# allisoneer/zvdb

Measured on NVIDIA B200. Metric: batched search QPS at recall@10 (1M x 128 fp32), higher is better.
Workload: dtype f32

## Files before the change

zvdb_b200/csrc/capi.cu:

```cuda
#include <cstring>
#include <algorithm>
#include <atomic>
#include <cstdio>
#include <cstdlib>
#include <mutex>
#include <new>
#include <string>
#include <vector>

#include "../../include/zvdb_b200.h"
#include "host_graph.hpp"
#include "search_kernel.cuh"
#include "search_team_kernel.cuh"
#include "builder.cuh"
#include "bruteforce.cuh"

namespace zvdb {

static thread_local std::string g_last_error;

static int fail(int code, const std::string &msg) {
    g_last_error = msg;
    return code;
}

#define ZV_CUDA(expr)                                                                            \
    do {                                                                                         \
        cudaError_t e__ = (expr);                                                                \
        if (e__ != cudaSuccess) {                                                                \
            cudaGetLastError();                                                                  \
            return fail(e__ == cudaErrorMemoryAllocation ? ZVDB_ERR_OUT_OF_MEMORY : ZVDB_ERR_CUDA, \
                        std::string(#expr) + ": " + cudaGetErrorString(e__));                    \
        }                                                                                        \
    } while (0)


__global__ void scatter_adj_rows_kernel(uint32_t *__restrict__ adj, const uint32_t *__restrict__ rows,
                                        const uint32_t *__restrict__ ids, uint32_t count, uint32_t m) {
    const uint64_t total = static_cast<uint64_t>(count) * m;
    for (uint64_t i = blockIdx.x * static_cast<uint64_t>(blockDim.x) + threadIdx.x; i < total;
         i += static_cast<uint64_t>(gridDim.x) * blockDim.x) {
        const uint32_t r = static_cast<uint32_t>(i / m), c = static_cast<uint32_t>(i % m);
        adj[static_cast<uint64_t>(ids[r]) * m + c] = rows[i];
    }
}

__global__ void arena_to_f16_kernel(uint2 *__restrict__ dst, const float4 *__restrict__ src, uint64_t r0, uint64_t r1,
                                    uint32_t row_chunks, uint32_t *__restrict__ bad_row) {
    const uint64_t begin = r0 * row_chunks, end = r1 * row_chunks;
    for (uint64_t i = begin + blockIdx.x * static_cast<uint64_t>(blockDim.x) + threadIdx.x; i < end;
         i += static_cast<uint64_t>(gridDim.x) * blockDim.x) {
        const float4 v = src[i];
        const __half2 a = __floats2half2_rn(v.x, v.y), b = __floats2half2_rn(v.z, v.w);
        if (__hisinf(__low2half(a)) | __hisinf(__high2half(a)) | __hisinf(__low2half(b)) | __hisinf(__high2half(b)))
            atomicMin(bad_row, static_cast<uint32_t>(i / row_chunks));
        dst[i] = make_uint2(*reinterpret_cast<const uint32_t *>(&a), *reinterpret_cast<const uint32_t *>(&b));
    }
}

template <typename T>
struct DevBuf {
    T *p = nullptr;
    size_t cap = 0;
    cudaError_t reserve(size_t count) {
        if (count <= cap) return cudaSuccess;
        if (p) cudaFree(p);
// ... 5 lines not shown
    void free_() { if (p) cudaFree(p); p = nullptr; cap = 0; }
};

}

using namespace zvdb;

struct zvdb_index {
    std::mutex mu;
    HostGraph g;
    int device = 0;
    int num_sms = 148;
    size_t smem_optin = 0;
    cudaStream_t stream = nullptr;
    cudaStream_t stream2 = nullptr;
    cudaStream_t stream_in = nullptr;
    cudaEvent_t in_ev[8] = {};
    cudaEvent_t bitmap_ev = nullptr;
    cudaEvent_t bf_ev = nullptr;
    unsigned char *h_stage = nullptr;
    size_t h_stage_cap = 0;
    uint32_t *mailbox_dev = nullptr;
    uint32_t mailbox_seq = 0;
    bool mailbox_armed = false;
    float *d_arena = nullptr;
    uint32_t *d_adj = nullptr;
    uint64_t cap_rows = 0, n_dev = 0;
    uint32_t cap_row_floats = 0, cap_m = 0;
    int storage = ZVDB_STORAGE_F32;
    uint2 *d_arena16 = nullptr;
    uint64_t f16_rows = 0;
    DevBuf<uint32_t> f16_bad;
    DevBuf<float> q_buf, dist_buf;
    DevBuf<uint64_t> ids_buf;
    DevBuf<uint32_t> cnt_buf, pops_buf, evals_buf, scat_rows, scat_ids, bitmap_buf, vlog_buf;
    DevBuf<uint64_t> res_buf;
    DevBuf<uint32_t> gtable_buf;
    DevBuf<float> bf_xhi, bf_xlo, bf_xnorm, bf_qhi, bf_qlo;
    DevBuf<uint64_t> bf_part, bf_glists;
    DevBuf<uint4> bf_segs;
    DevBuf<uint32_t> bf_seg_off;
    uint64_t bf_rows = 0;
    DevBuf<uint8_t> d_level;
    DevBuf<uint32_t> d_upper_base, d_upper_adj;
    DevBuf<uint4> seeds_buf;
    uint64_t upper_uploaded = ~0ull;
    bool descent = false;
    uint32_t visited_mode = 0;
    bool legacy_exchange = false;
    bool bitmap_oom = false;
    bool exchange_blocks = false;
    bool stage_host_buffers = false;
    uint32_t team_mode = 0;
    uint32_t prefetch_mode = 0;
    uint32_t bf_mode = 0;
    uint32_t bf_epilogue = 0;
    bool bf_filter = false;
    std::atomic<uint64_t> launches{0};
};

namespace zvdb {

static int ensure_capacity(zvdb_index *ix, uint64_t rows) {
    const HostGraph &g = ix->g;
    const bool same_layout = ix->cap_row_floats == g.row_floats && ix->cap_m == g.m;
    if (same_layout && rows <= ix->cap_rows) return ZVDB_OK;
    if (!same_layout) {
        ZV_CUDA(cudaDeviceSynchronize());
        cudaFree(ix->d_arena); cudaFree(ix->d_adj);
        ix->d_arena = nullptr; ix->d_adj = nullptr; ix->cap_rows = 0; ix->n_dev = 0; ix->bf_rows = 0;
        ix->cap_row_floats = g.row_floats; ix->cap_m = g.m;
    }
    if (ix->d_arena16) {
        ZV_CUDA(cudaDeviceSynchronize());
        cudaFree(ix->d_arena16); ix->d_arena16 = nullptr; ix->f16_rows = 0;
    }
    uint64_t nc = std::max<uint64_t>(rows, std::max<uint64_t>(ix->cap_rows * 2, 1024));
    float *na = nullptr; uint32_t *nj = nullptr;
    ZV_CUDA(cudaMalloc(&na, nc * g.row_floats * sizeof(float)));
    cudaError_t e = cudaMalloc(&nj, nc * g.m * sizeof(uint32_t));
    if (e != cudaSuccess) { cudaFree(na); ZV_CUDA(e); }
    if (ix->n_dev) {
        ZV_CUDA(cudaMemcpyAsync(na, ix->d_arena, ix->n_dev * g.row_floats * sizeof(float), cudaMemcpyDeviceToDevice, ix->stream));
        ZV_CUDA(cudaMemcpyAsync(nj, ix->d_adj, ix->n_dev * g.m * sizeof(uint32_t), cudaMemcpyDeviceToDevice, ix->stream));
        ZV_CUDA(cudaStreamSynchronize(ix->stream));
    }
    cudaFree(ix->d_arena); cudaFree(ix->d_adj);
    ix->d_arena = na; ix->d_adj = nj; ix->cap_rows = nc;
    return ZVDB_OK;
}

static int sync_device_locked(zvdb_index *ix) {
    HostGraph &g = ix->g;
    if (g.n == 0) return ZVDB_OK;
    if (g.rows_uploaded == g.n && !g.adj_all_dirty && g.dirty.empty()) return ZVDB_OK;
    ZV_CUDA(cudaSetDevice(ix->device));
    if (ix->n_dev) ZV_CUDA(cudaDeviceSynchronize());
    int rc = ensure_capacity(ix, g.n);
    if (rc) return rc;
    ix->f16_rows = std::min<uint64_t>(ix->f16_rows, g.rows_uploaded);
    for (uint64_t r = g.rows_uploaded; r < g.n;) {
        const uint64_t chunk = r / g.rows_per_chunk;
        const uint64_t end = std::min<uint64_t>(g.n, (chunk + 1) * g.rows_per_chunk);
        ZV_CUDA(cudaMemcpyAsync(ix->d_arena + r * g.row_floats, g.point(r), (end - r) * g.row_floats * sizeof(float),
                                cudaMemcpyHostToDevice, ix->stream));
        r = end;
// ... 128 lines not shown
    }
    return cudaGetLastError();
}
template <int ROWF>
static cudaError_t launch_descend_rowf(int metric, int cpl, const SearchParams &p, unsigned grid, cudaStream_t s) {
    switch (metric) {
        case 0: return launch_descend_metric<kMetricL2, ROWF>(cpl, p, grid, s);
        case 1: return launch_descend_metric<kMetricCos, ROWF>(cpl, p, grid, s);
        default: return launch_descend_metric<kMetricDot, ROWF>(cpl, p, grid, s);
    }
}
static cudaError_t launch_descend(bool f16, int metric, int cpl, const SearchParams &p, unsigned grid, cudaStream_t s) {
    return f16 ? launch_descend_rowf<kRowF16>(metric, cpl, p, grid, s) : launch_descend_rowf<kRowF32>(metric, cpl, p, grid, s);
}

template <int CPL, int METRIC, bool ADJC, int MC, int T, int ROWF>
static cudaError_t launch_team_inst3(const SearchParams &p, unsigned grid, size_t smem, cudaStream_t s) {
    auto kern = ROWF == kRowF16 ? search_team_f16_kernel<CPL, METRIC, ADJC, MC, T> : search_team_kernel<CPL, METRIC, ADJC, MC, T>;
    if (smem > 48 * 1024) {
        cudaError_t e = cudaFuncSetAttribute(kern, cudaFuncAttributeMaxDynamicSharedMemorySize, static_cast<int>(smem));
        if (e != cudaSuccess) return e;
    }
    kern<<<grid, T, smem, s>>>(p);
    return cudaGetLastError();
}
template <int CPL, int METRIC, int ROWF>
static cudaError_t launch_team_inst(bool adjc, unsigned threads, const SearchParams &p, unsigned grid, size_t smem, cudaStream_t s) {
    if (threads == 128) return launch_team_inst3<CPL, METRIC, false, 0, 128, ROWF>(p, grid, smem, s);
    if (adjc && p.m == 16) return launch_team_inst3<CPL, METRIC, true, 16, 256, ROWF>(p, grid, smem, s);
    return adjc ? launch_team_inst3<CPL, METRIC, true, 0, 256, ROWF>(p, grid, smem, s) : launch_team_inst3<CPL, METRIC, false, 0, 256, ROWF>(p, grid, smem, s);
}
template <int METRIC, int ROWF>
static cudaError_t launch_team_metric(int cpl, bool adjc, unsigned threads, const SearchParams &p, unsigned grid, size_t smem, cudaStream_t s) {
    switch (cpl) {
        case 1: return launch_team_inst<1, METRIC, ROWF>(adjc, threads, p, grid, smem, s);
        case 2: return launch_team_inst<2, METRIC, ROWF>(adjc, threads, p, grid, smem, s);
        case 4: return launch_team_inst<4, METRIC, ROWF>(adjc, threads, p, grid, smem, s);
        case 6: return launch_team_inst<6, METRIC, ROWF>(adjc, threads, p, grid, smem, s);
        case 8: return launch_team_inst<8, METRIC, ROWF>(adjc, threads, p, grid, smem, s);
    }
    return cudaErrorInvalidValue;
}
template <int ROWF>
static cudaError_t launch_team_rowf(int metric, int cpl, bool adjc, unsigned threads, const SearchParams &p, unsigned grid, size_t smem, cudaStream_t s) {
    switch (metric) {
        case 0: return launch_team_metric<kMetricL2, ROWF>(cpl, adjc, threads, p, grid, smem, s);
        case 1: return launch_team_metric<kMetricCos, ROWF>(cpl, adjc, threads, p, grid, smem, s);
        default: return launch_team_metric<kMetricDot, ROWF>(cpl, adjc, threads, p, grid, smem, s);
    }
}
static cudaError_t launch_team(bool f16, int metric, int cpl, bool adjc, unsigned threads, const SearchParams &p, unsigned grid, size_t smem, cudaStream_t s) {
    return f16 ? launch_team_rowf<kRowF16>(metric, cpl, adjc, threads, p, grid, smem, s)
               : launch_team_rowf<kRowF32>(metric, cpl, adjc, threads, p, grid, smem, s);
}

static int plan_visited(const zvdb_index *ix, uint32_t ef) {
    const HostGraph &g = ix->g;
    const uint64_t bound = std::min<uint64_t>(g.n, 1ull + static_cast<uint64_t>(ef) * g.m);
    const uint64_t slots = bound + bound / 4 + 16;
    const uint64_t cand_cap = std::max<uint64_t>(2, next_pow2(ef));
    const uint64_t smem_lists = (((static_cast<uint64_t>(ef) + 1) & ~1ull) + cand_cap) * 8 + kPoolCap * 8 + 32 * 4 + kPoolCap * 4 + 16;
    const uint64_t smem_hash = smem_lists + slots * 4;
    const uint64_t ctas = std::min<uint64_t>(32, (227ull * 1024) / (smem_hash + 1024));
    const uint64_t bitmap_bytes = (g.n + 31) / 32 * 4 * 32ull * static_cast<uint64_t>(ix->num_sms);
    int vis = (smem_hash <= ix->smem_optin && ctas >= 20) ? kVisSmemHash
            : ((bitmap_bytes <= (32ull << 30) && !ix->bitmap_oom) ? kVisGlobalBitmap : kVisGlobalHash);
    if (ix->visited_mode == 1) vis = kVisSmemHash;
    if (ix->visited_mode == 2) vis = kVisGlobalBitmap;
    if (ix->visited_mode == 3) vis = kVisGlobalHash;
    return vis;
}

struct FusedExchange {
    uint32_t *peer_qflags[8];
    const uint32_t *qflags;
    const uint8_t *gather;
    uint64_t block_bytes;
    uint64_t *m_ids; float *m_dist; uint32_t *m_counts;
    uint32_t world, rank, epoch;
    uint8_t *peer_ll[8] = {};
    const uint8_t *ll_local = nullptr;
    uint32_t ll_lines = 0, ll_pitch = 0, ll_nq = 0;
    uint32_t q_per = 0;
    const float *peer_q[8] = {};
    uint32_t *peer_sflags[8] = {};
    const uint32_t *sflags = nullptr;
    uint32_t sflag_pitch = 0;
};

static int launch_search(zvdb_index *ix, const float *d_q, uint64_t nq, uint32_t k, uint32_t ef, uint64_t *d_ids,
                         float *d_dist, uint32_t *d_counts, uint32_t *d_pops, uint32_t *d_evals, uint64_t id_stride,
                         uint64_t id_base, cudaStream_t s, uint8_t *const *peer_blocks = nullptr, uint32_t n_peers = 0,
                         const FusedExchange *fx = nullptr) {
    const HostGraph &g = ix->g;
    if (nq == 0) return ZVDB_OK;
    if (nq > 0x7FFFFFFFull) return fail(ZVDB_ERR_UNSUPPORTED, "nq exceeds 2^31-1 queries per launch");
    const bool f16 = ix->storage == ZVDB_STORAGE_F16 && g.n > 0;
    if (f16 && (fx || n_peers)) return fail(ZVDB_ERR_UNSUPPORTED, "f16 storage: the sharded exchange forms gather fp32 rows only");
    if (f16) {
        int rcf = sync_f16_locked(ix);
        if (rcf) return rcf;
    }
    SearchParams p{};
    p.arena = reinterpret_cast<const float4 *>(ix->d_arena);
    p.arena16 = f16 ? ix->d_arena16 : nullptr;
    p.adj = ix->d_adj;
// ... 16 lines not shown
            ZV_CUDA(ix->seeds_buf.reserve(nq));
        }
        p.seeds = ix->seeds_buf.p;
    }
    const uint32_t chunks_per_lane = (p.row_chunks + 31) / 32;
    if (chunks_per_lane > 8) return fail(ZVDB_ERR_UNSUPPORTED, "dim > 1024 is not built into the search kernel");
    const int cpl = chunks_per_lane <= 1 ? 1 : chunks_per_lane <= 2 ? 2 : chunks_per_lane <= 4 ? 4 : chunks_per_lane <= 6 ? 6 : 8;

    const uint64_t bound = std::max<uint64_t>(1, std::min<uint64_t>(g.n, 1ull + static_cast<uint64_t>(ef) * g.m));
    const uint64_t slots = bound + bound / 4 + 16;
    const uint64_t hash_words = (slots + 3) & ~3ull;
    const uint64_t cand_cap = std::max<uint64_t>(2, next_pow2(ef));
    const uint64_t smem_lists = (((static_cast<uint64_t>(ef) + 1) & ~1ull) + cand_cap) * 8 + kPoolCap * 8 + 32 * 4 + kPoolCap * 4 + 16;
    const uint64_t smem_hash = smem_lists + slots * 4;
    const bool team_auto = ix->team_mode == 0 && ix->visited_mode == 0 && ix->prefetch_mode == 0;
    if (!fx && n_peers == 0 && g.n > 0 && ef > 0 && (team_auto || ix->team_mode >= 2)) {
        const uint32_t ucpl = static_cast<uint32_t>(cpl);
        const uint64_t cap256 = team_cand_cap(ef, g.m, 256), cap128 = team_cand_cap(ef, g.m, 128);
        const uint64_t smem_plain = team_smem_bytes(cap256, ef, hash_words, ucpl, g.m, false);
        const uint64_t smem_cache = team_smem_bytes(cap256, ef, hash_words, ucpl, g.m, true);
        const uint64_t smem_half = team_smem_bytes(cap128, ef, hash_words, ucpl, g.m, false);
        const uint64_t regs256 = cpl <= 1 ? 3 : (cpl <= 4 ? 2 : 1);
        const uint64_t regs128 = cpl <= 1 ? 7 : (cpl <= 2 ? 6 : (cpl <= 4 ? 4 : 2));
        auto resident = [&](uint64_t smem, uint64_t by_regs) { return std::min<uint64_t>(by_regs, (227ull * 1024) / (smem + 1024)) * ix->num_sms; };
        const bool fits_cache = smem_cache <= ix->smem_optin, fits_plain = smem_plain <= ix->smem_optin, fits_half = smem_half <= ix->smem_optin;
        bool use = false, adjc = false;
        unsigned threads = 256;
        uint64_t team_cap = cap256, team_smem = smem_plain;
        if (ix->team_mode == 3) { use = fits_half; threads = 128; }
        else if (ix->team_mode == 2) { use = fits_plain; adjc = fits_cache && (nq <= resident(smem_cache, regs256) || resident(smem_cache, regs256) >= resident(smem_plain, regs256)); }
        else if (fits_cache && nq <= resident(smem_cache, regs256)) { use = true; adjc = true; }
        else if (fits_plain && nq <= resident(smem_plain, regs256)) { use = true; }
        else if (fits_half && nq <= resident(smem_half, regs128)) { use = true; threads = 128; }
        if (adjc) team_smem = smem_cache;
        if (threads == 128) { team_cap = cap128; team_smem = smem_half; }
        if (use) {
            cudaError_t e;
            if (p.seeds) {
                ZV_CUDA(cudaStreamWaitEvent(s, ix->bitmap_ev, 0));
                e = launch_descend(f16, g.metric, cpl, p, static_cast<unsigned>((nq + 3) / 4), s);
                ix->launches++;
                ZV_CUDA(e);
            }
            p.slots = static_cast<uint32_t>(slots); p.hash_words = static_cast<uint32_t>(hash_words);
            p.cand_cap = static_cast<uint32_t>(team_cap);
            if (ix->mailbox_dev && nq == 1) { p.done_flag = ix->mailbox_dev; p.done_seq = ix->mailbox_seq; ix->mailbox_armed = true; }
            e = launch_team(f16, g.metric, cpl, adjc, threads, p, static_cast<unsigned>(nq), static_cast<size_t>(team_smem), s);
            ix->launches++;
            ZV_CUDA(e);
            if (p.seeds) ZV_CUDA(cudaEventRecord(ix->bitmap_ev, s));
            return ZVDB_OK;
        }
    }
    uint64_t merge_smem = 0;
    if (fx) {
        const uint64_t total = static_cast<uint64_t>(fx->world) * k;
        if (total > 4096) return fail(ZVDB_ERR_UNSUPPORTED, "merge: G*k > 4096");
        p.merge_p2 = next_pow2(static_cast<uint32_t>(total));
        merge_smem = (total * 12 + 8 * 4 + 15) & ~15ull;
    }
    auto ctas_for = [](uint64_t smem) { return std::min<uint64_t>(32, (227ull * 1024) / (smem + 1024)); };
    int vis = plan_visited(ix, ef);
    if (vis == kVisGlobalBitmap && ix->visited_mode == 0) {
        const uint64_t resident0 = std::min<uint64_t>(nq, 32ull * ix->num_sms);
        const uint64_t need0 = resident0 * ((g.n + 31) / 32);
        if (need0 > ix->bitmap_buf.cap) {
            cudaError_t eb = ix->bitmap_buf.reserve(need0);
            if (eb == cudaErrorMemoryAllocation) { cudaGetLastError(); ix->bitmap_oom = true; vis = plan_visited(ix, ef); }
            else { ZV_CUDA(eb); ZV_CUDA(cudaMemsetAsync(ix->bitmap_buf.p, 0, ix->bitmap_buf.cap * sizeof(uint32_t), s)); }
        }
    }
    const uint64_t res_cap = (static_cast<uint64_t>(ef) + 1) & ~1ull;
    const bool res_global = vis != kVisSmemHash && ctas_for(smem_lists + merge_smem) < 32;
    uint64_t smem = vis == kVisSmemHash ? smem_hash : (res_global ? smem_lists - res_cap * 8 : smem_lists);
    smem = (smem + 15) & ~15ull;
    p.merge_off = static_cast<uint32_t>(smem);
    smem += merge_smem;
    if (smem > ix->smem_optin) {
        char buf[256];
        snprintf(buf, sizeof buf, "search needs %llu bytes of shared memory per query (ef=%u, m=%u); this device allows %zu. Lower ef.",
                 static_cast<unsigned long long>(smem), ef, g.m, ix->smem_optin);
        return fail(ZVDB_ERR_UNSUPPORTED, buf);
    }
    p.slots = static_cast<uint32_t>(slots); p.hash_words = static_cast<uint32_t>(hash_words);
    p.prefetch = ix->prefetch_mode == 0 ? ((vis != kVisSmemHash && cpl <= 2) ? 1u : 0u) : ix->prefetch_mode - 1u;
    p.cand_cap = static_cast<uint32_t>(cand_cap);
    const uint64_t resident = std::min<uint64_t>(ctas_for(smem), cpl <= 2 ? 32 : 16) * ix->num_sms;
    unsigned grid = static_cast<unsigned>(nq);
    if (vis != kVisSmemHash) {
        grid = static_cast<unsigned>(std::min<uint64_t>(nq, resident));
        ZV_CUDA(cudaStreamWaitEvent(s, ix->bitmap_ev, 0));
        if (vis == kVisGlobalBitmap) {
            const uint64_t bm_words = (g.n + 31) / 32;
            const uint64_t need = grid * bm_words;
            if (need > ix->bitmap_buf.cap) {
                ZV_CUDA(ix->bitmap_buf.reserve(need));
                ZV_CUDA(cudaMemsetAsync(ix->bitmap_buf.p, 0, ix->bitmap_buf.cap * sizeof(uint32_t), s));
            }
            const uint64_t log_cap = (bound + 3) & ~3ull;
            ZV_CUDA(ix->vlog_buf.reserve(grid * log_cap));
            p.gbitmap = ix->bitmap_buf.p; p.glog = ix->vlog_buf.p;
            p.bm_words = static_cast<uint32_t>(bm_words); p.log_cap = static_cast<uint32_t>(log_cap);
        } else {
            const uint64_t need = grid * hash_words;
            if (need > ix->gtable_buf.cap) {
                ZV_CUDA(ix->gtable_buf.reserve(need));
                ZV_CUDA(cudaMemsetAsync(ix->gtable_buf.p, 0xFF, ix->gtable_buf.cap * sizeof(uint32_t), s));
            }
            p.gtable = ix->gtable_buf.p;
        }
        if (res_global) {
            ZV_CUDA(ix->res_buf.reserve(grid * res_cap));
            p.gres = ix->res_buf.p; p.res_cap = static_cast<uint32_t>(res_cap);
        }
// ... 336 lines not shown
    fp.id_stride = id_stride; fp.id_base = id_base;
    fp.row_chunks = pitch / 4; fp.dim = g.dim; fp.nq = p.nq; fp.k = k; fp.kp = p.kp; fp.n_splits = p.n_slots;
    fp.p2 = next_pow2(p.n_slots * p.kp); fp.kk2 = std::max<uint32_t>(2, next_pow2(p.kp));
    const uint32_t cpl_raw = (fp.row_chunks + 31) / 32;
    const int cpl = cpl_raw <= 1 ? 1 : cpl_raw <= 2 ? 2 : cpl_raw <= 4 ? 4 : cpl_raw <= 6 ? 6 : 8;
    const size_t fsmem = (static_cast<size_t>(fp.p2) + fp.kk2) * sizeof(uint64_t);
    cudaError_t e = g.metric == 0 ? launch_bf_final_metric<kMetricL2>(cpl, fp, fsmem, s)
                  : g.metric == 1 ? launch_bf_final_metric<kMetricCos>(cpl, fp, fsmem, s)
                                  : launch_bf_final_metric<kMetricDot>(cpl, fp, fsmem, s);
    ix->launches++;
    ZV_CUDA(e);
    ZV_CUDA(cudaEventRecord(ix->bf_ev, s));
    return ZVDB_OK;
}

}


extern "C" {

const char *zvdb_last_error(void) { return g_last_error.c_str(); }
const char *zvdb_version(void) { return "zvdb_b200 0.1 sm_100a"; }

int zvdb_create(zvdb_index **out, uint32_t dim, uint32_t m, uint32_t ef_construction, int metric, int device) {
    if (!out) return fail(ZVDB_ERR_INVALID, "zvdb_create: out is null");
    *out = nullptr;
    if (m == 0) return fail(ZVDB_ERR_INVALID, "zvdb_create: m must be >= 1");
    if (metric < 0 || metric > 2) return fail(ZVDB_ERR_INVALID, "zvdb_create: unknown metric");
    if (dim > 1024) return fail(ZVDB_ERR_UNSUPPORTED, "zvdb_create: dim > 1024 is not built into the search kernel");
    int count = 0;
    cudaError_t e = cudaGetDeviceCount(&count);
    if (e != cudaSuccess || device < 0 || device >= count) {
        cudaGetLastError();
        return fail(ZVDB_ERR_CUDA, std::string("zvdb_create: no usable CUDA device (there is no CPU fallback): ") +
                                       (e != cudaSuccess ? cudaGetErrorString(e) : "device ordinal out of range"));
    }
    cudaDeviceProp prop{};
    ZV_CUDA(cudaGetDeviceProperties(&prop, device));
    if (prop.major != 10)
        return fail(ZVDB_ERR_CUDA, std::string("zvdb_create: device '") + prop.name + "' is not sm_100; this library carries sm_100a code only");
    zvdb_index *ix = new (std::nothrow) zvdb_index();
    if (!ix) return fail(ZVDB_ERR_OUT_OF_MEMORY, "zvdb_create: out of memory");
    ix->device = device;
    ix->num_sms = prop.multiProcessorCount;
    ix->smem_optin = prop.sharedMemPerBlockOptin;
    ix->g.m = m; ix->g.ef_construction = ef_construction; ix->g.metric = metric;
    if (dim) ix->g.fix_dim(dim);
    e = cudaSetDevice(device);
    if (e == cudaSuccess) e = cudaStreamCreateWithFlags(&ix->stream, cudaStreamNonBlocking);
    if (e == cudaSuccess) e = cudaStreamCreateWithFlags(&ix->stream2, cudaStreamNonBlocking);
    if (e == cudaSuccess) e = cudaStreamCreateWithFlags(&ix->stream_in, cudaStreamNonBlocking);
    for (int i = 0; i < 8 && e == cudaSuccess; ++i) e = cudaEventCreateWithFlags(&ix->in_ev[i], cudaEventDisableTiming);
    if (e == cudaSuccess) e = cudaEventCreateWithFlags(&ix->bitmap_ev, cudaEventDisableTiming);
    if (e == cudaSuccess) e = cudaEventCreateWithFlags(&ix->bf_ev, cudaEventDisableTiming);
    if (e != cudaSuccess) { delete ix; ZV_CUDA(e); }
    *out = ix;
    return ZVDB_OK;
}

void zvdb_destroy(zvdb_index *ix) {
    if (!ix) return;
    cudaSetDevice(ix->device);
    if (ix->stream) { cudaStreamSynchronize(ix->stream); cudaStreamDestroy(ix->stream); }
    if (ix->stream2) { cudaStreamSynchronize(ix->stream2); cudaStreamDestroy(ix->stream2); }
    if (ix->stream_in) { cudaStreamSynchronize(ix->stream_in); cudaStreamDestroy(ix->stream_in); }
    for (int i = 0; i < 8; ++i) if (ix->in_ev[i]) cudaEventDestroy(ix->in_ev[i]);
    if (ix->bitmap_ev) cudaEventDestroy(ix->bitmap_ev);
    if (ix->bf_ev) cudaEventDestroy(ix->bf_ev);
    cudaFree(ix->d_arena); cudaFree(ix->d_adj); cudaFree(ix->d_arena16);
    if (ix->h_stage) cudaFreeHost(ix->h_stage);
    ix->f16_bad.free_();
    ix->q_buf.free_(); ix->dist_buf.free_(); ix->ids_buf.free_(); ix->cnt_buf.free_();
    ix->pops_buf.free_(); ix->evals_buf.free_(); ix->scat_rows.free_(); ix->scat_ids.free_(); ix->bitmap_buf.free_(); ix->vlog_buf.free_(); ix->res_buf.free_(); ix->gtable_buf.free_();
    ix->d_level.free_(); ix->d_upper_base.free_(); ix->d_upper_adj.free_(); ix->seeds_buf.free_();
    ix->bf_xhi.free_(); ix->bf_xlo.free_(); ix->bf_xnorm.free_(); ix->bf_qhi.free_(); ix->bf_qlo.free_(); ix->bf_part.free_(); ix->bf_glists.free_(); ix->bf_segs.free_(); ix->bf_seg_off.free_();
    delete ix;
}

int zvdb_set_level_seed(zvdb_index *ix, uint64_t seed) {
    if (!ix) return fail(ZVDB_ERR_INVALID, "null index");
    std::lock_guard<std::mutex> lk(ix->mu);
    ix->g.rng = seed * 0x9E3779B97F4A7C15ull + 0x243F6A8885A308D3ull;
    return ZVDB_OK;
}

static void to_f32(const void *src, uint64_t count, int dtype, float *dst) {
    if (dtype == 1) { const double *p = static_cast<const double *>(src); for (uint64_t i = 0; i < count; ++i) dst[i] = static_cast<float>(p[i]); }
    else if (dtype == 2) { const int32_t *p = static_cast<const int32_t *>(src); for (uint64_t i = 0; i < count; ++i) dst[i] = static_cast<float>(p[i]); }
    else std::memcpy(dst, src, count * sizeof(float));
}

static int insert_locked(zvdb_index *ix, const void *points_any, uint64_t n, uint32_t dim, const int32_t *levels, int dtype = 0) {
    HostGraph &g = ix->g;
    if (n == 0) return ZVDB_OK;
    if (!points_any) return fail(ZVDB_ERR_INVALID, "insert: null point");
    if (dtype < 0 || dtype > 2) return fail(ZVDB_ERR_INVALID, "insert: dtype must be 0 (f32), 1 (f64) or 2 (i32)");
    if (g.n == 0 && g.chunks.empty()) g.dtype = dtype;
    if (dtype != g.dtype) return fail(ZVDB_ERR_INVALID, "insert: element type differs from the index's (one HNSW(T) holds one T)");
    if (dtype != 0 && g.metric != 0) return fail(ZVDB_ERR_UNSUPPORTED, "insert: f64 / i32 indexes are squared-L2 only, like the reference");
    const float *points = static_cast<const float *>(points_any);
    if (g.dim == 0) {
        if (dim == 0) return fail(ZVDB_ERR_INVALID, "insert: dim must be >= 1");
        if (dim > 1024) return fail(ZVDB_ERR_UNSUPPORTED, "insert: dim > 1024 is not built into the search kernel");
        g.fix_dim(dim);
    }
    if (dim != g.dim) return fail(ZVDB_ERR_DIM_MISMATCH, "Mismatched dimensions in distance calculation");
    cudaSetDevice(ix->device);
    if (dtype == 0) {
        for (uint64_t i = 0; i < n; ++i) {
            if (g.insert(points + i * static_cast<uint64_t>(dim), levels ? levels[i] : -1))
                return fail(ZVDB_ERR_OUT_OF_MEMORY, "insert: out of memory");
        }
        return ZVDB_OK;
    }
    std::vector<float> conv(dim);
    const size_t es = g.elem_size();
    for (uint64_t i = 0; i < n; ++i) {
        const unsigned char *src = static_cast<const unsigned char *>(points_any) + i * static_cast<uint64_t>(dim) * es;
        to_f32(src, dim, dtype, conv.data());
        if (g.insert(conv.data(), levels ? levels[i] : -1, src)) return fail(ZVDB_ERR_OUT_OF_MEMORY, "insert: out of memory");
    }
    return ZVDB_OK;
}

int zvdb_insert(zvdb_index *ix, const float *point, uint32_t dim) {
    if (!ix) return fail(ZVDB_ERR_INVALID, "null index");
// ... 446 lines not shown
    ZV_CUDA(cudaGetLastError());
    const uint64_t total = n * g.m;
    const unsigned blocks = static_cast<unsigned>(std::min<uint64_t>((total + 255) / 256, 148ull * 16));
    count_reverse_kernel<<<blocks, 256, 0, s>>>(d_fw.p, total, d_indeg.p); ix->launches++;
    std::vector<uint32_t> indeg;
    std::vector<uint64_t> off;
    try { indeg.resize(n); off.resize(n + 1); }
    catch (const std::bad_alloc &) { return fail(ZVDB_ERR_OUT_OF_MEMORY, "build: out of memory"); }
    ZV_CUDA(cudaMemcpyAsync(indeg.data(), d_indeg.p, n * sizeof(uint32_t), cudaMemcpyDeviceToHost, s));
    ZV_CUDA(cudaStreamSynchronize(s));
    off[0] = 0;
    for (uint64_t i = 0; i < n; ++i) off[i + 1] = off[i] + indeg[i];
    ZV_CUDA(d_rev.reserve(std::max<uint64_t>(off[n], 1)));
    ZV_CUDA(cudaMemcpyAsync(d_off.p, off.data(), (n + 1) * sizeof(uint64_t), cudaMemcpyHostToDevice, s));
    fill_reverse_kernel<<<blocks, 256, 0, s>>>(d_fw.p, total, g.m, d_off.p, d_indeg.p + n, d_rev.p); ix->launches++;
    bp.rev_off = d_off.p; bp.rev = d_rev.p;
    launch_build(g.metric, cpl, 3, bp, s); ix->launches++;
    ZV_CUDA(cudaGetLastError());
    ZV_CUDA(cudaMemcpyAsync(g.adj0.data(), ix->d_adj, n * g.m * sizeof(uint32_t), cudaMemcpyDeviceToHost, s));
    ZV_CUDA(cudaStreamSynchronize(s));
    return ZVDB_OK;
}

int zvdb_build_from_candidates(zvdb_index *ix, const float *points, uint64_t n, uint32_t dim, const uint32_t *cand,
                               uint32_t K, int cand_on_device) {
    if (!ix || (n && (!points || !cand))) return fail(ZVDB_ERR_INVALID, "null argument");
    if (K == 0 || K > kBuildBuf) return fail(ZVDB_ERR_UNSUPPORTED, "build: K must be in 1..128");
    std::lock_guard<std::mutex> lk(ix->mu);
    HostGraph &g = ix->g;
    if (g.m > 64) return fail(ZVDB_ERR_UNSUPPORTED, "build: m must be <= 64");
    int rc = set_points_locked(ix, points, n, dim, 0);
    if (rc || n == 0) return rc;
    rc = build_from_candidates_locked(ix, n, cand, K, cand_on_device);
    if (rc) {
        const std::string why = g_last_error;
        g.reset_nodes();
        ix->n_dev = 0; ix->bf_rows = 0; ix->f16_rows = 0;
        return fail(rc, why);
    }
    g.rows_uploaded = n; g.dirty.clear(); g.adj_all_dirty = false;
    ix->n_dev = n;
    return ZVDB_OK;
}

int zvdb_sync_device(zvdb_index *ix) {
    if (!ix) return fail(ZVDB_ERR_INVALID, "null index");
    std::lock_guard<std::mutex> lk(ix->mu);
    return sync_device_locked(ix);
}

int zvdb_set_kernel_variant(zvdb_index *ix, uint32_t variant) {
    if (!ix) return fail(ZVDB_ERR_INVALID, "null index");
    const uint32_t width = variant & 3u, vis = (variant >> 2) & 3u, bfm = (variant >> 4) & 3u;
    if (width > 2 || bfm > 2 || variant > 65535 || ((variant >> 8) & 7u) > 4)
        return fail(ZVDB_ERR_INVALID, "variant: bits 0-1 = accepted and ignored (round 1's load-width variants are gone: never faster in any automatically chosen mode), bits 2-3 = visited set 0 auto/1 shared-memory hash/2 global bitmap/3 global hash, bits 4-5 = brute force 0 auto/1 single CTA/2 CTA pair, bit 6 = brute-force TF32 filter, bit 7 = brute-force sorted-list epilogue, bits 8-10 = L2 prefetch 0 auto/1 off/2 rows/3 adjacency/4 both, bit 11 = stage page-locked host buffers through device copies, bit 12 = sharded step as three launches (search, flag, merge) instead of the fused one, bit 13 = fused step through result blocks + release flags instead of 128-byte records, bits 14-15 = one CTA per query for small batches 0 auto/1 never/2 full teams (256 threads) whenever the shape fits/3 half teams (128 threads)");
    std::lock_guard<std::mutex> lk(ix->mu);
    ix->prefetch_mode = (variant >> 8) & 7u; ix->stage_host_buffers = (variant >> 11) & 1u; ix->legacy_exchange = (variant >> 12) & 1u; ix->exchange_blocks = (variant >> 13) & 1u;
    ix->team_mode = (variant >> 14) & 3u;
    ix->visited_mode = vis; ix->bf_mode = bfm; ix->bf_filter = (variant >> 6) & 1u; ix->bf_epilogue = (variant >> 7) & 1u;
    return ZVDB_OK;
}

uint64_t zvdb_kernel_launches(const zvdb_index *ix) { return ix ? ix->launches.load() : 0; }

int zvdb_search_batch_device(zvdb_index *ix, const float *d_queries, uint64_t nq, uint32_t k, uint32_t ef,
                             uint64_t *d_ids, float *d_dist, uint32_t *d_counts, uint32_t *d_pops, uint32_t *d_evals,
                             uint64_t id_stride, uint64_t id_base, void *stream) {
    if (!ix) return fail(ZVDB_ERR_INVALID, "null index");
    if (nq == 0) return ZVDB_OK;
    if (!d_queries || !d_ids || !d_dist || !d_counts) return fail(ZVDB_ERR_INVALID, "search: null buffer");
    if (k == 0) return fail(ZVDB_ERR_INVALID, "search: k must be >= 1");
    if (ef == 0) ef = k;
    if (ef < k) return fail(ZVDB_ERR_INVALID, "search: ef must be >= k");
    std::lock_guard<std::mutex> lk(ix->mu);
    ZV_CUDA(cudaSetDevice(ix->device));
    cudaStream_t s = static_cast<cudaStream_t>(stream);
    if (ix->g.n == 0 || !ix->g.has_entry) {
        ZV_CUDA(cudaMemsetAsync(d_counts, 0, nq * sizeof(uint32_t), s));
        ZV_CUDA(cudaMemsetAsync(d_ids, 0xFF, nq * k * sizeof(uint64_t), s));
        ZV_CUDA(cudaMemsetAsync(d_dist, 0, nq * k * sizeof(float), s));
        if (d_pops) ZV_CUDA(cudaMemsetAsync(d_pops, 0, nq * sizeof(uint32_t), s));
        if (d_evals) ZV_CUDA(cudaMemsetAsync(d_evals, 0, nq * sizeof(uint32_t), s));
        return ZVDB_OK;
    }
    int rc = sync_device_locked(ix);
    if (rc) return rc;
    return launch_search(ix, d_queries, nq, k, ef, d_ids, d_dist, d_counts, d_pops, d_evals, id_stride, id_base, s);
}

int zvdb_search_batch(zvdb_index *ix, const float *queries, uint64_t nq, uint32_t dim, uint32_t k, uint32_t ef,
                      uint64_t *ids, float *dist, uint32_t *counts, uint32_t *pops, uint32_t *evals) {
    if (!ix) return fail(ZVDB_ERR_INVALID, "null index");
    if (nq == 0) return ZVDB_OK;
    if (!queries || !ids || !dist || !counts) return fail(ZVDB_ERR_INVALID, "search: null buffer");
    if (k == 0) return fail(ZVDB_ERR_INVALID, "search: k must be >= 1");
    if (ef == 0) ef = k;
    if (ef < k) return fail(ZVDB_ERR_INVALID, "search: ef must be >= k");
    std::lock_guard<std::mutex> lk(ix->mu);
    ZV_CUDA(cudaSetDevice(ix->device));
    if (ix->g.n == 0 || !ix->g.has_entry) {
        for (uint64_t i = 0; i < nq; ++i) counts[i] = 0;
        for (uint64_t i = 0; i < nq * k; ++i) { ids[i] = ZVDB_INVALID_ID; dist[i] = 0.0f; }
        if (pops) for (uint64_t i = 0; i < nq; ++i) pops[i] = 0;
        if (evals) for (uint64_t i = 0; i < nq; ++i) evals[i] = 0;
        return ZVDB_OK;
    }
    if (dim != ix->g.dim) return fail(ZVDB_ERR_DIM_MISMATCH, "Mismatched dimensions in distance calculation");
    int rc = sync_device_locked(ix);
    if (rc) return rc;
    auto mapped = [](const void *ptr, void **dptr) {
        cudaPointerAttributes a{};
// ... 433 lines not shown
```

zvdb_b200/csrc/search_kernel.cuh:

```cuda
#pragma once
#include <cuda_fp16.h>
#include <type_traits>
#include "common.cuh"

namespace zvdb {

struct SearchParams {
    const float4 *arena;
    const uint32_t *adj;
    const float *queries;
    uint64_t *ids;
    float *dist;
    uint32_t *counts;
    uint32_t *pops;
    uint32_t *evals;
    uint64_t id_stride, id_base;
    uint32_t row_chunks;
    uint32_t m, n, entry, dim, nq, k, ef;
    uint32_t slots;
    uint32_t hash_words;
    uint32_t cand_cap;
    uint8_t *peer_blocks[8];
    uint32_t n_peers;
    const uint8_t *levels;
    const uint32_t *upper_base;
    const uint32_t *upper_adj;
    uint32_t max_level, descent_start;
    uint4 *seeds;
    uint32_t *gbitmap;
    uint32_t *glog;
    uint32_t bm_words, log_cap;
    uint64_t *gres;
    uint32_t res_cap;
    uint32_t prefetch;
    uint32_t *gtable;
    uint32_t *peer_qflags[8];
    const uint32_t *qflags;
    const uint8_t *gather;
    uint64_t block_bytes;
    uint64_t *m_ids; float *m_dist; uint32_t *m_counts;
    uint32_t ex_world, ex_rank, ex_epoch;
    uint32_t merge_p2;
    uint32_t merge_lag;
    uint32_t merge_off;
    uint8_t *peer_ll[8];
    const uint8_t *ll_local;
    uint32_t ll_lines;
    uint32_t ll_pitch;
    uint32_t ll_nq;
    uint32_t q_per;
    const float *peer_q[8];
    uint32_t *peer_sflags[8];
    const uint32_t *sflags;
    uint32_t sflag_pitch;
    uint32_t *done_flag;
    uint32_t done_seq;
    const uint2 *arena16;
};

enum : int { kMetricL2 = 0, kMetricCos = 1, kMetricDot = 2 };
constexpr uint32_t kPoolCap = 64;

enum : int { kRowF32 = 0, kRowF16 = 1 };
template <int ROWF> using RowChunk = std::conditional_t<ROWF == kRowF16, uint2, float4>;
__device__ __forceinline__ float4 chunk_f32(const float4 v) { return v; }
__device__ __forceinline__ float4 chunk_f32(const uint2 w) {
    const float2 a = __half22float2(*reinterpret_cast<const __half2 *>(&w.x));
    const float2 b = __half22float2(*reinterpret_cast<const __half2 *>(&w.y));
    return make_float4(a.x, a.y, b.x, b.y);
}
template <int ROWF> __device__ __forceinline__ RowChunk<ROWF> zero_chunk() {
    if constexpr (ROWF == kRowF16) return make_uint2(0u, 0u); else return make_float4(0.f, 0.f, 0.f, 0.f);
}
template <int ROWF> __device__ __forceinline__ const RowChunk<ROWF> *search_rows(const SearchParams &p) {
    if constexpr (ROWF == kRowF16) return p.arena16; else return p.arena;
}

#ifndef ZVDB_F16_UNROLL
#define ZVDB_F16_UNROLL 1
#endif
template <int CPL, bool WIDE, int ROWF = kRowF32> struct Unroll {
    static constexpr int narrow = CPL <= 1 ? 8 : (CPL <= 2 ? 4 : 2);
    static constexpr int value = (WIDE ? (CPL <= 4 ? narrow * 2 : narrow) : narrow) * (ROWF == kRowF16 ? ZVDB_F16_UNROLL : 1);
};

__device__ __forceinline__ uint64_t pack2(float lo, float hi) {
    uint64_t r; asm("mov.b64 %0, {%1, %2};" : "=l"(r) : "f"(lo), "f"(hi)); return r;
}
__device__ __forceinline__ void unpack2(uint64_t v, float &lo, float &hi) {
    asm("mov.b64 {%0, %1}, %2;" : "=f"(lo), "=f"(hi) : "l"(v));
}
__device__ __forceinline__ uint64_t ffma2(uint64_t a, uint64_t b, uint64_t c) {
    uint64_t d; asm("fma.rn.f32x2 %0, %1, %2, %3;" : "=l"(d) : "l"(a), "l"(b), "l"(c)); return d;
}

struct Chunk2 { uint64_t xy, zw; };

template <int METRIC>
__device__ __forceinline__ uint64_t accumulate_chunk(uint64_t acc, const Chunk2 q, const float4 v) {
    const uint64_t vxy = pack2(v.x, v.y), vzw = pack2(v.z, v.w);
    if (METRIC == kMetricL2) {
        const uint64_t neg1 = pack2(-1.0f, -1.0f);
        const uint64_t dxy = ffma2(vxy, neg1, q.xy);
        const uint64_t dzw = ffma2(vzw, neg1, q.zw);
        acc = ffma2(dxy, dxy, acc);
        acc = ffma2(dzw, dzw, acc);
    } else {
        acc = ffma2(q.xy, vxy, acc);
        acc = ffma2(q.zw, vzw, acc);
    }
// ... 671 lines not shown
```

Before: 23.55 million.

## Add two-queries-per-warp search kernel with small on-chip visited table

Adds a new graph search kernel in which each warp serves two queries, one per 16-lane half. Each half keeps its own candidate list, pool and a small shared-memory visited hash, and spills to a global hash table when linear probing overflows. The kernel is chosen automatically for L2 f32 batches with degree up to 16 when the shared-memory hash path would apply, with the aim of packing more queries per SM and cutting per-query shared memory. The cost is that the two halves run in lockstep, so the warp keeps iterating until both queries finish, and overflow falls back to slower global atomics.

Measured after the change: 16.41 million (median of 6 runs). 0.697x the previous value.

```diff
diff --git a/zvdb_b200/csrc/capi.cu b/zvdb_b200/csrc/capi.cu
--- a/zvdb_b200/csrc/capi.cu
+++ b/zvdb_b200/csrc/capi.cu
@@ -12,6 +12,7 @@
 #include "host_graph.hpp"
 #include "search_kernel.cuh"
 #include "search_team_kernel.cuh"
+#include "search_pair_kernel.cuh"
 #include "builder.cuh"
 #include "bruteforce.cuh"
 
@@ -123,6 +124,11 @@
     bool exchange_blocks = false;
     bool stage_host_buffers = false;
     uint32_t team_mode = 0;
+    bool pair_off = false;
+    bool pair_tiny = false;
+    DevBuf<uint64_t> pair_res2;
+    DevBuf<uint32_t> pair_tab2;
+    cudaEvent_t pair_ev2 = nullptr;
     uint32_t prefetch_mode = 0;
     uint32_t bf_mode = 0;
     uint32_t bf_epilogue = 0;
@@ -357,6 +363,15 @@
 static cudaError_t launch_team(bool f16, int metric, int cpl, bool adjc, unsigned threads, const SearchParams &p, unsigned grid, size_t smem, cudaStream_t s) {
     return f16 ? launch_team_rowf<kRowF16>(metric, cpl, adjc, threads, p, grid, smem, s)
                : launch_team_rowf<kRowF32>(metric, cpl, adjc, threads, p, grid, smem, s);
+}
+
+static cudaError_t launch_pair(const SearchParams &p, unsigned grid, size_t smem, cudaStream_t s) {
+    if (smem > 48 * 1024) {
+        cudaError_t e = cudaFuncSetAttribute(search_pair_kernel<kMetricL2>, cudaFuncAttributeMaxDynamicSharedMemorySize, static_cast<int>(smem));
+        if (e != cudaSuccess) return e;
+    }
+    search_pair_kernel<kMetricL2><<<grid, 32, smem, s>>>(p);
+    return cudaGetLastError();
 }
 
 static int plan_visited(const zvdb_index *ix, uint32_t ef) {
@@ -479,6 +494,43 @@
             return ZVDB_OK;
         }
     }
+    auto ctas_for = [](uint64_t smem) { return std::min<uint64_t>(32, (227ull * 1024) / (smem + 1024)); };
+    if (!fx && n_peers == 0 && !f16 && g.n > 0 && ef > 0 && cpl == 1 && g.m <= 16 && g.metric == 0 && !ix->pair_off && ix->prefetch_mode == 0 &&
+        plan_visited(ix, ef) == kVisSmemHash) {
+        uint64_t pslots = 64;
+        while (pslots * 2 <= bound && !ix->pair_tiny) pslots *= 2;
+        const uint64_t per_q = pair_query_smem(cand_cap, pslots), psmem = 2 * per_q;
+        const uint64_t pctas = ctas_for(psmem);
+        if (psmem <= ix->smem_optin && 2 * pctas >= ctas_for((smem_hash + 15) & ~15ull)) {
+            const bool second = s == ix->stream2 && !p.seeds;
+            DevBuf<uint64_t> &rbuf = second ? ix->pair_res2 : ix->res_buf;
+            DevBuf<uint32_t> &tbuf = second ? ix->pair_tab2 : ix->gtable_buf;
+            cudaEvent_t ev = second ? ix->pair_ev2 : ix->bitmap_ev;
+            const unsigned grid = static_cast<unsigned>(std::min<uint64_t>((nq + 1) / 2, pctas * ix->num_sms));
+            const uint64_t res_cap = (static_cast<uint64_t>(ef) + 1) & ~1ull;
+            ZV_CUDA(cudaStreamWaitEvent(s, ev, 0));
+            ZV_CUDA(rbuf.reserve(2ull * grid * res_cap));
+            if (2ull * grid * hash_words > tbuf.cap) {
+                ZV_CUDA(tbuf.reserve(2ull * grid * hash_words));
+                ZV_CUDA(cudaMemsetAsync(tbuf.p, 0xFF, tbuf.cap * sizeof(uint32_t), s));
+            }
+            p.gres = rbuf.p; p.res_cap = static_cast<uint32_t>(res_cap);
+            p.gtable = tbuf.p; p.slots = static_cast<uint32_t>(slots); p.hash_words = static_cast<uint32_t>(hash_words);
+            p.cand_cap = static_cast<uint32_t>(cand_cap);
+            p.pair_slots = static_cast<uint32_t>(pslots); p.pair_stride = static_cast<uint32_t>(per_q);
+            cudaError_t e;
+            if (p.seeds) {
+                e = launch_descend(false, g.metric, cpl, p, static_cast<unsigned>((nq + 3) / 4), s);
+                ix->launches++;
+                ZV_CUDA(e);
+            }
+            e = launch_pair(p, grid, static_cast<size_t>(psmem), s);
+            ix->launches++;
+            ZV_CUDA(e);
+            ZV_CUDA(cudaEventRecord(ev, s));
+            return ZVDB_OK;
+        }
+    }
     uint64_t merge_smem = 0;
     if (fx) {
         const uint64_t total = static_cast<uint64_t>(fx->world) * k;
@@ -486,7 +538,6 @@
         p.merge_p2 = next_pow2(static_cast<uint32_t>(total));
         merge_smem = (total * 12 + 8 * 4 + 15) & ~15ull;
     }
-    auto ctas_for = [](uint64_t smem) { return std::min<uint64_t>(32, (227ull * 1024) / (smem + 1024)); };
     int vis = plan_visited(ix, ef);
     if (vis == kVisGlobalBitmap && ix->visited_mode == 0) {
         const uint64_t resident0 = std::min<uint64_t>(nq, 32ull * ix->num_sms);
@@ -929,6 +980,7 @@
     if (e == cudaSuccess) e = cudaStreamCreateWithFlags(&ix->stream_in, cudaStreamNonBlocking);
     for (int i = 0; i < 8 && e == cudaSuccess; ++i) e = cudaEventCreateWithFlags(&ix->in_ev[i], cudaEventDisableTiming);
     if (e == cudaSuccess) e = cudaEventCreateWithFlags(&ix->bitmap_ev, cudaEventDisableTiming);
+    if (e == cudaSuccess) e = cudaEventCreateWithFlags(&ix->pair_ev2, cudaEventDisableTiming);
     if (e == cudaSuccess) e = cudaEventCreateWithFlags(&ix->bf_ev, cudaEventDisableTiming);
     if (e != cudaSuccess) { delete ix; ZV_CUDA(e); }
     *out = ix;
@@ -943,12 +995,14 @@
     if (ix->stream_in) { cudaStreamSynchronize(ix->stream_in); cudaStreamDestroy(ix->stream_in); }
     for (int i = 0; i < 8; ++i) if (ix->in_ev[i]) cudaEventDestroy(ix->in_ev[i]);
     if (ix->bitmap_ev) cudaEventDestroy(ix->bitmap_ev);
+    if (ix->pair_ev2) cudaEventDestroy(ix->pair_ev2);
     if (ix->bf_ev) cudaEventDestroy(ix->bf_ev);
     cudaFree(ix->d_arena); cudaFree(ix->d_adj); cudaFree(ix->d_arena16);
     if (ix->h_stage) cudaFreeHost(ix->h_stage);
     ix->f16_bad.free_();
     ix->q_buf.free_(); ix->dist_buf.free_(); ix->ids_buf.free_(); ix->cnt_buf.free_();
     ix->pops_buf.free_(); ix->evals_buf.free_(); ix->scat_rows.free_(); ix->scat_ids.free_(); ix->bitmap_buf.free_(); ix->vlog_buf.free_(); ix->res_buf.free_(); ix->gtable_buf.free_();
+    ix->pair_res2.free_(); ix->pair_tab2.free_();
     ix->d_level.free_(); ix->d_upper_base.free_(); ix->d_upper_adj.free_(); ix->seeds_buf.free_();
     ix->bf_xhi.free_(); ix->bf_xlo.free_(); ix->bf_xnorm.free_(); ix->bf_qhi.free_(); ix->bf_qlo.free_(); ix->bf_part.free_(); ix->bf_glists.free_(); ix->bf_segs.free_(); ix->bf_seg_off.free_();
     delete ix;
@@ -1501,11 +1555,12 @@
 int zvdb_set_kernel_variant(zvdb_index *ix, uint32_t variant) {
     if (!ix) return fail(ZVDB_ERR_INVALID, "null index");
     const uint32_t width = variant & 3u, vis = (variant >> 2) & 3u, bfm = (variant >> 4) & 3u;
-    if (width > 2 || bfm > 2 || variant > 65535 || ((variant >> 8) & 7u) > 4)
-        return fail(ZVDB_ERR_INVALID, "variant: bits 0-1 = accepted and ignored (round 1's load-width variants are gone: never faster in any automatically chosen mode), bits 2-3 = visited set 0 auto/1 shared-memory hash/2 global bitmap/3 global hash, bits 4-5 = brute force 0 auto/1 single CTA/2 CTA pair, bit 6 = brute-force TF32 filter, bit 7 = brute-force sorted-list epilogue, bits 8-10 = L2 prefetch 0 auto/1 off/2 rows/3 adjacency/4 both, bit 11 = stage page-locked host buffers through device copies, bit 12 = sharded step as three launches (search, flag, merge) instead of the fused one, bit 13 = fused step through result blocks + release flags instead of 128-byte records, bits 14-15 = one CTA per query for small batches 0 auto/1 never/2 full teams (256 threads) whenever the shape fits/3 half teams (128 threads)");
+    if (width > 2 || bfm > 2 || variant > 0x3FFFFu || ((variant >> 8) & 7u) > 4)
+        return fail(ZVDB_ERR_INVALID, "variant: bits 0-1 = accepted and ignored (round 1's load-width variants are gone: never faster in any automatically chosen mode), bits 2-3 = visited set 0 auto/1 shared-memory hash/2 global bitmap/3 global hash, bits 4-5 = brute force 0 auto/1 single CTA/2 CTA pair, bit 6 = brute-force TF32 filter, bit 7 = brute-force sorted-list epilogue, bits 8-10 = L2 prefetch 0 auto/1 off/2 rows/3 adjacency/4 both, bit 11 = stage page-locked host buffers through device copies, bit 12 = sharded step as three launches (search, flag, merge) instead of the fused one, bit 13 = fused step through result blocks + release flags instead of 128-byte records, bits 14-15 = one CTA per query for small batches 0 auto/1 never/2 full teams (256 threads) whenever the shape fits/3 half teams (128 threads), bit 16 = never two queries per warp, bit 17 = two queries per warp with a 64-slot on-chip visited table");
     std::lock_guard<std::mutex> lk(ix->mu);
     ix->prefetch_mode = (variant >> 8) & 7u; ix->stage_host_buffers = (variant >> 11) & 1u; ix->legacy_exchange = (variant >> 12) & 1u; ix->exchange_blocks = (variant >> 13) & 1u;
     ix->team_mode = (variant >> 14) & 3u;
+    ix->pair_off = (variant >> 16) & 1u; ix->pair_tiny = (variant >> 17) & 1u;
     ix->visited_mode = vis; ix->bf_mode = bfm; ix->bf_filter = (variant >> 6) & 1u; ix->bf_epilogue = (variant >> 7) & 1u;
     return ZVDB_OK;
 }
diff --git a/zvdb_b200/csrc/search_kernel.cuh b/zvdb_b200/csrc/search_kernel.cuh
--- a/zvdb_b200/csrc/search_kernel.cuh
+++ b/zvdb_b200/csrc/search_kernel.cuh
@@ -56,6 +56,7 @@
     uint32_t *done_flag;
     uint32_t done_seq;
     const uint2 *arena16;
+    uint32_t pair_stride, pair_slots;
 };
 
 enum : int { kMetricL2 = 0, kMetricCos = 1, kMetricDot = 2 };
diff --git a/zvdb_b200/csrc/search_pair_kernel.cuh b/zvdb_b200/csrc/search_pair_kernel.cuh
--- /dev/null
+++ b/zvdb_b200/csrc/search_pair_kernel.cuh
@@ -0,0 +1,270 @@
+#pragma once
+#include "search_team_kernel.cuh"
+
+namespace zvdb {
+
+constexpr uint32_t kPairProbes = 8;
+constexpr int kPairU = 4;
+
+__host__ __device__ inline uint64_t pair_query_smem(uint64_t cand_cap, uint64_t slots) {
+    return cand_cap * 8 + kPoolCap * 8 + 16 * 4 + slots * 4;
+}
+
+__device__ __forceinline__ bool pair_visited_insert(uint32_t *table, uint32_t slots, uint32_t id, const SearchParams &p,
+                                                    uint32_t owner, bool &ovf) {
+    uint32_t s = __umulhi(id * 0x9E3779B1u, slots);
+#pragma unroll 1
+    for (uint32_t i = 0; i < kPairProbes; ++i) {
+        const uint32_t prev = atomicCAS(table + s, kInvalidId, id);
+        if (prev == kInvalidId) return true;
+        if (prev == id) return false;
+        s = (s + 1u) & (slots - 1u);
+    }
+    ovf = true;
+    return visited_insert(p.gtable + static_cast<size_t>(owner) * p.hash_words, p.slots, id);
+}
+
+__device__ __forceinline__ void load_half_query(Chunk2 &qlo, Chunk2 &qhi, const float *__restrict__ qp, uint32_t dim, uint32_t j) {
+    const bool vec = (dim & 3u) == 0 && (reinterpret_cast<uintptr_t>(qp) & 15u) == 0;
+#pragma unroll
+    for (int c = 0; c < 2; ++c) {
+        const uint32_t i = (j + 16u * c) * 4u;
+        float4 v = make_float4(0.f, 0.f, 0.f, 0.f);
+        if (vec) {
+            if (i < dim) v = *reinterpret_cast<const float4 *>(qp + i);
+        } else {
+            v.x = i + 0 < dim ? qp[i + 0] : 0.f; v.y = i + 1 < dim ? qp[i + 1] : 0.f;
+            v.z = i + 2 < dim ? qp[i + 2] : 0.f; v.w = i + 3 < dim ? qp[i + 3] : 0.f;
+        }
+        Chunk2 &q = c ? qhi : qlo;
+        q.xy = pack2(v.x, v.y); q.zw = pack2(v.z, v.w);
+    }
+}
+
+template <int METRIC>
+__device__ __forceinline__ float pair_rows_distance(const float4 *__restrict__ arena, uint32_t row_chunks, const uint32_t (&ids)[kPairU],
+                                                    const Chunk2 &qlo, const Chunk2 &qhi, uint32_t j, uint32_t lane) {
+    float4 vlo[kPairU], vhi[kPairU];
+    if (row_chunks == 32u) {
+        const char *__restrict__ b = reinterpret_cast<const char *>(arena + j);
+#pragma unroll
+        for (int u = 0; u < kPairU; ++u) {
+            const float4 *__restrict__ row = reinterpret_cast<const float4 *>(b + static_cast<uint64_t>(ids[u]) * 512u);
+            vlo[u] = __ldg(row);
+            vhi[u] = __ldg(row + 16);
+        }
+    } else {
+#pragma unroll
+        for (int u = 0; u < kPairU; ++u) {
+            const float4 *__restrict__ row = arena + static_cast<size_t>(ids[u]) * row_chunks;
+            vlo[u] = make_float4(0.f, 0.f, 0.f, 0.f); vhi[u] = vlo[u];
+            if (j < row_chunks) vlo[u] = __ldg(row + j);
+            if (j + 16u < row_chunks) vhi[u] = __ldg(row + j + 16u);
+        }
+    }
+    float acc[kPairU];
+#pragma unroll
+    for (int u = 0; u < kPairU; ++u)
+        acc[u] = __fadd_rn(lane_partial(accumulate_chunk<METRIC>(0ull, qlo, vlo[u])), lane_partial(accumulate_chunk<METRIC>(0ull, qhi, vhi[u])));
+    transposed_reduce<kPairU>(acc, lane, 8);
+    return finish_distance<METRIC>(acc[0]);
+}
+
+__device__ __forceinline__ void pair_bitonic_sort(uint64_t *a, uint32_t p2, uint32_t j) {
+    for (uint32_t size = 2; size <= p2; size <<= 1) {
+        for (uint32_t stride = size >> 1; stride > 0; stride >>= 1) {
+            __syncwarp();
+            for (uint32_t i = j; i < (p2 >> 1); i += 16) {
+                const uint32_t lo = 2 * i - (i & (stride - 1)), hi = lo + stride;
+                const bool up = (lo & size) == 0;
+                const uint64_t x = a[lo], y = a[hi];
+                if ((y < x) == up && x != y) { a[lo] = y; a[hi] = x; }
+            }
+        }
+    }
+    __syncwarp();
+}
+
+__device__ __forceinline__ uint32_t pair_merge_pool(uint64_t *win, uint32_t ns, uint32_t cap, uint64_t *pool, uint32_t npool, uint32_t j) {
+    for (uint32_t t = npool + j; t < kPoolCap; t += 16) pool[t] = ~0ull;
+    pair_bitonic_sort(pool, kPoolCap, j);
+    uint32_t pos[kPoolCap / 16];
+#pragma unroll
+    for (int r = 0; r < static_cast<int>(kPoolCap / 16); ++r) {
+        const uint32_t t = j + 16u * r;
+        pos[r] = kInvalidId;
+        if (t < npool) {
+            const uint32_t re = lower_bound_u64(win, ns, pool[t]);
+            if (re + t < cap) pos[r] = re + t;
+        }
+    }
+    const uint32_t lo = npool ? lower_bound_u64(win, ns, pool[0]) : ns;
+    const uint32_t n_it = (ns - lo + 15u) / 16u;
+    const uint32_t n_max = max(n_it, __shfl_xor_sync(kFullMask, n_it, 16));
+    for (uint32_t it = 0; it < n_max; ++it) {
+        const uint32_t hi = ns - 16u * it;
+        const bool active = it < n_it && hi - lo > j;
+        const uint32_t i = hi - 1u - j;
+        uint64_t e = 0; uint32_t s = 0;
+        if (active) { e = win[i]; s = lower_bound_u64(pool, npool, e); }
+        __syncwarp();
+        if (active && i + s < cap) win[i + s] = e;
+    }
+    __syncwarp();
+#pragma unroll
+    for (int r = 0; r < static_cast<int>(kPoolCap / 16); ++r) if (pos[r] != kInvalidId) win[pos[r]] = pool[j + 16u * r];
+    __syncwarp();
+    return min(ns + npool, cap);
+}
+
+template <int METRIC>
+__global__ void __launch_bounds__(32, 32)
+search_pair_kernel(const __grid_constant__ SearchParams p) {
+    extern __shared__ __align__(16) unsigned char smem_raw[];
+    const uint32_t lane = threadIdx.x, half = lane >> 4, j = lane & 15u, hshift = half * 16u;
+    const uint32_t owner = blockIdx.x * 2u + half;
+    uint64_t *cand = reinterpret_cast<uint64_t *>(smem_raw + half * p.pair_stride);
+    uint64_t *pool = cand + p.cand_cap;
+    uint32_t *todo = reinterpret_cast<uint32_t *>(pool + kPoolCap);
+    uint32_t *table = todo + 16;
+    uint64_t *res = p.gres + static_cast<size_t>(owner) * p.res_cap;
+    const float4 *__restrict__ arena = p.arena;
+
+    for (uint32_t pair = blockIdx.x; pair * 2u < p.nq; pair += gridDim.x) {
+    const uint32_t q = pair * 2u + half;
+    const bool has_q = q < p.nq;
+    const uint32_t qq = has_q ? q : q - 1u;
+    Chunk2 qlo[1], qhi[1];
+    load_half_query(qlo[0], qhi[0], p.queries + static_cast<size_t>(qq) * p.dim, p.dim, j);
+    for (uint32_t i = j; i < p.pair_slots / 4u; i += 16)
+        reinterpret_cast<uint4 *>(table)[i] = make_uint4(kInvalidId, kInvalidId, kInvalidId, kInvalidId);
+    __syncwarp();
+
+    bool live = has_q, ovf = false;
+    uint32_t np = 0, h = 0, ns = 0, npool = has_q ? 1u : 0u, nev = 1;
+    {
+        uint32_t entry = p.entry;
+        float d0;
+        if (p.seeds == nullptr) {
+            float4 vlo[1], vhi[1];
+            half_row_load<1, METRIC>(vlo, vhi, arena, p.row_chunks, entry, j);
+            d0 = half_row_reduce<1, METRIC>(vlo, vhi, qlo, qhi);
+        } else {
+            const uint4 sd = __ldg(p.seeds + qq);
+            entry = sd.x; d0 = __uint_as_float(sd.y);
+        }
+        if (has_q && j == 0) {
+            pool[0] = pack_key(d0, entry);
+            pair_visited_insert(table, p.pair_slots, entry, p, owner, ovf);
+        }
+    }
+    uint64_t worst = ~0ull;
+    uint32_t pref_id = kInvalidId, pref_nb = kInvalidId;
+    __syncwarp();
+
+    while (__any_sync(kFullMask, live)) {
+        uint64_t pk = ~0ull;
+        uint32_t pk_slot = 0;
+        if (live) {
+#pragma unroll
+            for (int r = 0; r < static_cast<int>(kPoolCap / 16); ++r) {
+                const uint32_t t = j + 16u * r;
+                if (t < npool) { const uint64_t x = pool[t]; if (x < pk) { pk = x; pk_slot = t; } }
+            }
+        }
+        const uint32_t pk_d = static_cast<uint32_t>(pk >> 32);
+        const uint32_t d_lo = __reduce_min_sync(kFullMask, half ? kInvalidId : pk_d);
+        const uint32_t d_hi = __reduce_min_sync(kFullMask, half ? pk_d : kInvalidId);
+        const uint32_t pmin_d = half ? d_hi : d_lo;
+        const uint32_t pk_i = pk_d == pmin_d ? static_cast<uint32_t>(pk) : kInvalidId;
+        const uint32_t i_lo = __reduce_min_sync(kFullMask, half ? kInvalidId : pk_i);
+        const uint32_t i_hi = __reduce_min_sync(kFullMask, half ? pk_i : kInvalidId);
+        const uint64_t pmin = (static_cast<uint64_t>(pmin_d) << 32) | (half ? i_hi : i_lo);
+        const uint64_t head = (live && ns > 0) ? cand[h] : ~0ull;
+        const uint64_t cur_key = min(head, pmin);
+        if (cur_key == ~0ull) live = false;
+        if (live) {
+            if (head <= pmin) { ++h; --ns; }
+            else {
+                if (pk == pmin) pool[pk_slot] = pool[npool - 1];
+                --npool;
+            }
+            if (j == 0) res[np] = cur_key;
+            ++np;
+        }
+        const uint32_t cur = live ? key_id(cur_key) : p.entry;
+        const uint32_t cap = p.ef - np;
+        if (ns > cap) ns = cap;
+        if (ns < cap) worst = ~0ull;
+        __syncwarp();
+
+        if (__any_sync(kFullMask, live && npool + p.m > kPoolCap)) {
+            ns = pair_merge_pool(cand + h, ns, cap, pool, live ? npool : 0u, j);
+            if (live) { npool = 0; worst = (ns == cap && ns > 0) ? cand[h + ns - 1] : ~0ull; }
+        }
+        uint32_t nb = kInvalidId;
+        if (live && j < p.m) nb = cur == pref_id ? pref_nb : __ldg(p.adj + static_cast<size_t>(cur) * p.m + j);
+        pref_id = (live && ns > 0) ? key_id(cand[h]) : kInvalidId;
+        pref_nb = (pref_id != kInvalidId && j < p.m) ? __ldg(p.adj + static_cast<size_t>(pref_id) * p.m + j) : kInvalidId;
+
+        bool fresh = false;
+        if (nb != kInvalidId) fresh = pair_visited_insert(table, p.pair_slots, nb, p, owner, ovf);
+        const unsigned ball = __ballot_sync(kFullMask, fresh);
+        const unsigned mask = (ball >> hshift) & 0xFFFFu;
+        const uint32_t t = __popc(mask);
+        const uint32_t tmax = max(__popc(ball & 0xFFFFu), __popc(ball >> 16));
+        if (tmax != 0) {
+            const uint32_t slot_t = __popc(mask & ((1u << j) - 1u));
+            if (fresh) todo[slot_t] = nb;
+            else todo[j - slot_t + t] = cur;
+            nev += t;
+            __syncwarp();
+
+            for (uint32_t j0 = 0; j0 < tmax; j0 += kPairU) {
+                const uint4 w = *reinterpret_cast<const uint4 *>(todo + j0);
+                const uint32_t ids[kPairU] = {w.x, w.y, w.z, w.w};
+                const float d = pair_rows_distance<METRIC>(arena, p.row_chunks, ids, qlo[0], qhi[0], j, lane);
+                const uint32_t r = j >> 2;
+                uint64_t key = ~0ull;
+                if ((j & 3u) == 0 && j0 + r < t) key = pack_key(d, todo[j0 + r]);
+                const bool keep = key < worst;
+                const unsigned km = (__ballot_sync(kFullMask, keep) >> hshift) & 0xFFFFu;
+                if (keep) pool[npool + __popc(km & ((1u << j) - 1u))] = key;
+                npool += __popc(km);
+            }
+        }
+        __syncwarp();
+        live = live && np < p.ef;
+    }
+
+    uint64_t *sorted = cand;
+    const uint32_t p2 = next_pow2(max(np, __shfl_xor_sync(kFullMask, np, 16)));
+    for (uint32_t i = j; i < p2; i += 16) sorted[i] = i < np ? ((res[i] & 0xFFFFFFFF00000000ull) | i) : ~0ull;
+    pair_bitonic_sort(sorted, p2, j);
+    if (has_q) {
+        const uint32_t nres = min(np, p.k);
+        for (uint32_t r = j; r < p.k; r += 16) {
+            const size_t o = static_cast<size_t>(q) * p.k + r;
+            uint64_t oid = ~0ull; float od = 0.0f;
+            if (r < nres) {
+                const uint64_t key = res[static_cast<uint32_t>(sorted[r])];
+                oid = static_cast<uint64_t>(key_id(key)) * p.id_stride + p.id_base;
+                od = key_dist(key);
+            }
+            p.ids[o] = oid; p.dist[o] = od;
+        }
+        if (j == 0) {
+            p.counts[q] = nres;
+            if (p.pops) p.pops[q] = np;
+            if (p.evals) p.evals[q] = nev + (p.seeds ? __ldg(p.seeds + q).z : 0u);
+        }
+    }
+    if ((__ballot_sync(kFullMask, ovf) >> hshift) & 0xFFFFu) {
+        uint4 *t4 = reinterpret_cast<uint4 *>(p.gtable + static_cast<size_t>(owner) * p.hash_words);
+        for (uint32_t i = j; i < p.hash_words / 4u; i += 16) t4[i] = make_uint4(kInvalidId, kInvalidId, kInvalidId, kInvalidId);
+    }
+    __syncwarp();
+    }
+}
+
+}
```
